# akloetgen/PARA-suite

Measured on AMD Instinct MI355X. Metric: aligned reads/sec (10Mx50bp PAR-CLIP vs hg19-size genome) on MI355X; SAM bit-exact vs own CPU restatement (parity unpinned), higher is better.
Workload: dtype u64

## Files before the change

para-suite_amd/csrc/ps_core.h:

```cpp
#pragma once
#include "ps_types.h"

namespace ps {

PS_HD uint32_t ps_popc(uint32_t x)
{
#ifdef __HIP_DEVICE_COMPILE__
    return (uint32_t)__popc(x);
#else
    return (uint32_t)__builtin_popcount(x);
#endif
}
PS_HD uint32_t pfx_mask32(int ns)
{
    return ns >= 32 ? 0xFFFFFFFFu : (ns <= 0 ? 0u : ((1u << ns) - 1u));
}

struct Blk { uint32_t x[16]; };

#ifdef __HIP_DEVICE_COMPILE__
#define PS_AS_GLOBAL(T, p) ((const __attribute__((address_space(1))) T *)(p))
#define PS_AS_GLOBAL_W(T, p) ((__attribute__((address_space(1))) T *)(p))
typedef uint32_t ps_u32x4 __attribute__((ext_vector_type(4)));
typedef uint32_t ps_u32x2 __attribute__((ext_vector_type(2)));
// ... 147 lines not shown
{
    if (base < 4) {
        uint32_t ok, ol;
        occ_pair1(ix, c.k, c.l, base, ok, ol, st);
        const bwtint l2 = L2_of(ix, base);
        c.k = l2 + ok + 1;
        c.l = l2 + ol;
    }
    if (c.k > c.l || base > 3) { c.k = 0; c.l = ix.seq_len; ++c.bid; }
    uint32_t w = width32(c.k, c.l);
    w_out = w;
    cw_out = cw_pack(c.bid, !first && w == c.prev_w);
    c.prev_w = w;
}

static const int PS_POP_TRIES = 1;
enum { M_FETCH = 0, M_POP = 1, M_EXACT = 2, M_EXPAND = 3, M_EXIT = 4, M_HIT = 5,
       M_GROW = 6 };

struct BtLane {
    int r, mode;
    bwtint k, l;
    int i, score, units, n_mm, n_gapo, n_gape, n_ins, n_del, state, ldp;
    bool have_cur;
    int best_score, max_units, n_aln, n_stack, status;
    unsigned long long best_cnt;
    unsigned long long bm0, bm1;
    uint32_t bump, free_head, iters0;
    uint32_t rn0, rn1;
    int len;
    uint32_t n_phantom;
    uint32_t cap;
    LaneStats st;
};

PS_HD int lm_ncw(int len) { return (len + 1 + 3) >> 2; }
PS_HD int lm_ncsw(int seed_len) { return seed_len > 0 ? (seed_len + 1 + 3) >> 2 : 0; }
PS_HD bool lm_nmask_in_regs(int len) { return len <= 64; }
PS_HD int lm_heads_off(int len, int seed_len) { return 4 * (lm_ncw(len) + lm_ncsw(seed_len) + ((len + 15) >> 4) + (lm_nmask_in_regs(len) ? 0 : ((len + 31) >> 5))); }
PS_HD int lm_bytes(int len, int seed_len, int n_buckets, bool wide)
{
    int n = lm_heads_off(len, seed_len) + (wide ? 0 : 2 * n_buckets);
    n = (n + 3) & ~3;
    if (((n >> 2) & 1) == 0) n += 4;
    return n;
}

static const int PS_JUMP_SLOT_WORDS = 8, PS_JUMP_MAX_LEVELS = 14;
PS_HD uint32_t jump_level_off(int d) { return 0x55555555u & ((1u << (2 * d)) - 1u); }
PS_HD size_t jump_words(int levels) { return (size_t)jump_level_off(levels) * PS_JUMP_SLOT_WORDS; }
PS_HD int jump_levels_for(bwtint seq_len) { int k = 0; while (k < PS_JUMP_MAX_LEVELS && (seq_len >> (2 * k)) >= 48) ++k; return k; }

static const int PS_CHASE_MIN2 = 16;
struct BtHot {
    const OccBlock *blocks; bwtint primary;
    const uint32_t *jump; uint32_t jump_levels;
    uint32_t skip_levels;
    uint32_t L2lo[4], L2hi;
    uint32_t s_pk[5], u_pk[5];
    uint32_t p0, p1, p2, p3;
    uint32_t inv_c_min, max_entries, pool_cap, n_reads, big_cap;
    uint32_t c_min;
    uint32_t chase;
    PS_HD int len() const { return (int)(p0 & 0xffu); }
    PS_HD int seed_len() const { return (int)((p0 >> 8) & 0xffu); }
    PS_HD int indel_end_skip() const { return (int)((p0 >> 16) & 0xffu); }
    PS_HD int max_del_occ() const { return (int)(p0 >> 24); }
    PS_HD int max_gapo() const { return (int)(p1 & 0xfu); }
    PS_HD int max_gape() const { return (int)((p1 >> 4) & 0xfu); }
    PS_HD bool mode_gape() const { return ((p1 >> 8) & 1u) != 0; }
    PS_HD bool use_seed() const { return ((p1 >> 9) & 1u) != 0; }
    PS_HD bool profile() const { return ((p1 >> 10) & 1u) != 0; }
    PS_HD bool has_big() const { return ((p1 >> 11) & 1u) != 0; }
    PS_HD int seed_units() const { return (int)((p1 >> 12) & 0xfffu); }
    PS_HD int u_tight() const { return (int)(p1 >> 24); }
    PS_HD int s_gapo_ins() const { return (int)(p2 & 0xffu); }
    PS_HD int s_gape() const { return (int)((p2 >> 8) & 0xffu); }
    PS_HD int s_gapo_del() const { return (int)((p2 >> 16) & 0xffu); }
    PS_HD int s_stop() const { return (int)(p2 >> 24); }
    PS_HD int u_gapo_ins() const { return (int)(p3 & 0xffu); }
    PS_HD int u_gape() const { return (int)((p3 >> 8) & 0xffu); }
    PS_HD int u_gapo_del() const { return (int)((p3 >> 16) & 0xffu); }
    PS_HD int n_buckets() const { return (int)(p3 >> 24); }
    PS_HD bwtint L2(int c) const
    { return (bwtint)L2lo[c] | ((bwtint)((L2hi >> c) & 1u) << 32); }
    PS_HD bwtint L2_dyn(int c) const
    { return (bwtint)sel4s(L2lo[0], L2lo[1], L2lo[2], L2lo[3], c) | ((bwtint)((L2hi >> c) & 1u) << 32); }
};
inline bool bt_hot_make(const BtArgs &a, BtHot &h)
{
    const Model &md = a.md;
    h.blocks = a.ix.blocks; h.primary = a.ix.primary; h.L2hi = 0;
    h.jump = a.ix.jump; h.jump_levels = a.ix.jump ? (uint32_t)a.ix.jump_levels : 0u;
    h.skip_levels = (a.no_skip || (((uint32_t)md.max_units * (uint32_t)md.inv_c_min) >> 16) > 127u) ? 0u : h.jump_levels;
    for (int c = 0; c < 4; ++c) { h.L2lo[c] = (uint32_t)a.ix.L2[c]; h.L2hi |= (uint32_t)((a.ix.L2[c] >> 32) & 1ull) << c; }
    h.L2hi |= (uint32_t)((a.ix.seq_len >> 32) & 1ull) << 4;
    for (int c = 0; c < 5; ++c) { h.s_pk[c] = md.s_mm_pk[c]; h.u_pk[c] = md.u_mm_pk[c]; }
    const int seed_units = md.max_seed_diff * md.u_tight;
    const bool ok = a.len >= 0 && a.len <= 255 && md.seed_len >= 0 && md.seed_len <= 255 && md.indel_end_skip >= 0 && md.indel_end_skip <= 255 &&
                    md.max_del_occ >= 0 && md.max_del_occ <= 255 && md.max_gapo >= 0 && md.max_gapo <= 15 && md.max_gape >= 0 && md.max_gape <= 15 &&
                    seed_units >= 0 && seed_units <= 4095 && md.u_tight >= 0 && md.u_tight <= 255 && md.s_stop >= 0 && md.s_stop <= 255 &&
                    md.s_gapo_ins >= 0 && md.s_gapo_ins <= 255 && md.s_gape >= 0 && md.s_gape <= 255 && md.s_gapo_del >= 0 && md.s_gapo_del <= 255 &&
                    md.u_gapo_ins >= 0 && md.u_gapo_ins <= 255 && md.u_gape >= 0 && md.u_gape <= 255 && md.u_gapo_del >= 0 && md.u_gapo_del <= 255 &&
                    md.n_buckets >= 0 && md.n_buckets <= 255 && md.max_entries >= 0 && md.inv_c_min >= 0 && md.max_units <= 255 && a.ix.L2[0] == 0;
    h.p0 = (uint32_t)a.len | ((uint32_t)md.seed_len << 8) | ((uint32_t)md.indel_end_skip << 16) | ((uint32_t)md.max_del_occ << 24);
    h.p1 = (uint32_t)md.max_gapo | ((uint32_t)md.max_gape << 4) | ((md.mode_gape ? 1u : 0u) << 8) | ((md.use_seed ? 1u : 0u) << 9) |
           ((md.profile ? 1u : 0u) << 10) | ((a.n_big ? 1u : 0u) << 11) | ((uint32_t)seed_units << 12) | ((uint32_t)md.u_tight << 24);
    h.p2 = (uint32_t)md.s_gapo_ins | ((uint32_t)md.s_gape << 8) | ((uint32_t)md.s_gapo_del << 16) | ((uint32_t)md.s_stop << 24);
    h.p3 = (uint32_t)md.u_gapo_ins | ((uint32_t)md.u_gape << 8) | ((uint32_t)md.u_gapo_del << 16) | ((uint32_t)md.n_buckets << 24);
    h.c_min = (uint32_t)md.c_min;
    h.chase = a.no_chase ? 0u : (uint32_t)(a.chase_min2 > 0 ? a.chase_min2 : PS_CHASE_MIN2);
    h.inv_c_min = (uint32_t)md.inv_c_min; h.max_entries = (uint32_t)md.max_entries; h.pool_cap = a.pool_cap; h.n_reads = (uint32_t)a.n_reads; h.big_cap = a.big_cap;
    return ok;
}

struct BtMem {
    uint8_t *cw, *csw;
    uint32_t *rb, *rn;
    uint16_t *heads16;
    void *pool;
    uint32_t *heads;
};

PS_HD void bt_mem_bind(BtMem &m, uint8_t *mine, int len, int seed_len)
{
    m.cw = mine; m.csw = mine + 4 * lm_ncw(len);
    m.rb = reinterpret_cast<uint32_t *>(m.csw + 4 * lm_ncsw(seed_len));
    m.rn = m.rb + ((len + 15) >> 4);
    m.heads16 = reinterpret_cast<uint16_t *>(mine + lm_heads_off(len, seed_len));
}
PS_HD int seq_at(const BtMem &m, const BtLane &L, int j, int len, int max_len)
{
    const int p = len - 1 - j;
    const uint32_t b = (m.rb[p >> 4] >> (2 * (p & 15))) & 3u;
    const uint32_t nw = lm_nmask_in_regs(max_len) ? (p < 32 ? L.rn0 : L.rn1) : m.rn[p >> 5];
    return ((nw >> (p & 31)) & 1u) ? 4 : 3 - (int)b;
}

struct Entry16 { uint32_t k, l, a, b; };
static const uint32_t PS_NIL16 = 0xFFFFu;

PS_HD bool bm_test(const BtLane &L, int b) { return (((b & 64) ? L.bm1 : L.bm0) >> (b & 63)) & 1ull; }
PS_HD void bm_set(BtLane &L, int b) { const unsigned long long v = 1ull << (b & 63); if (b & 64) L.bm1 |= v; else L.bm0 |= v; }
PS_HD void bm_clr(BtLane &L, int b) { const unsigned long long v = ~(1ull << (b & 63)); if (b & 64) L.bm1 &= v; else L.bm0 &= v; }
PS_HD int bm_first(const BtLane &L)
{
#ifdef __HIP_DEVICE_COMPILE__
    return L.bm0 ? (__ffsll((unsigned long long)L.bm0) - 1) : (64 + __ffsll((unsigned long long)L.bm1) - 1);
#else
    return L.bm0 ? __builtin_ctzll(L.bm0) : 64 + __builtin_ctzll(L.bm1);
#endif
}
PS_HD void store16(Entry16 *dst, const Entry16 &e)
{
#ifdef __HIP_DEVICE_COMPILE__
    ps_u32x4 v; v.x = e.k; v.y = e.l; v.z = e.a; v.w = e.b;
    *PS_AS_GLOBAL_W(ps_u32x4, dst) = v;
#else
    *dst = e;
#endif
}
PS_HD void load16(const Entry16 *src, Entry16 &e)
{
#ifdef __HIP_DEVICE_COMPILE__
// ... 346 lines not shown
```

para-suite_amd/csrc/ps_kernels.hip:

```cpp
#include <hip/hip_runtime.h>
#include <algorithm>
#include <cstdlib>
#include <stdexcept>
#include <string>
#include "ps_core.h"
#include "ps_narrow.h"
#include "ps_kernels.h"

namespace ps {

static const int PS_Q_CHUNK = 64;
#ifndef PS_BT_WAVES
#define PS_BT_WAVES 4
#endif

__device__ __forceinline__ unsigned long long wave_sum(unsigned long long v)
{
    for (int o = 32; o > 0; o >>= 1) v += __shfl_xor(v, o, 64);
    return v;
}
__device__ __forceinline__ void flush_stats(KStats *ks, const LaneStats &st)
{
    if (!ks) return;
    unsigned long long v[8] = {st.pairs, st.same, st.nodes, st.pushes, st.pops, st.lf, st.iters, st.exact};
// ... 21 lines not shown
        if (!seed_role) {
#pragma unroll 1
            for (int i = 0; i < len; ++i) {
                int j = len - 1 - i;
                if (i == 0 || (j & 15) == 15) bw = a.bases[(size_t)(j >> 4) * a.n_reads + opaque_lane(r)];
                if (i == 0 || (j & 31) == 31) mw = a.nmask[(size_t)(j >> 5) * a.n_reads + opaque_lane(r)];
                int base = ((mw >> (j & 31)) & 1u) ? 4 : (int)((bw >> (2 * (j & 15))) & 3u);
                uint32_t wv; uint8_t cb;
                wchain_step(a.ix, C, base, wv, cb, i == 0, st);
                a.w[(size_t)i * a.n_reads + opaque_lane(r)] = wv;
                cww |= (uint32_t)cb << (8 * (i & 3));
                if ((i & 3) == 3) { a.cwb[(size_t)(i >> 2) * a.n_reads + opaque_lane(r)] = cww; cww = 0; }
            }
            a.w[(size_t)len * a.n_reads + opaque_lane(r)] = 0;
            cww |= (uint32_t)cw_pack(C.bid + 1, false) << (8 * (len & 3));
            a.cwb[(size_t)(len >> 2) * a.n_reads + opaque_lane(r)] = cww;
        } else if (seeded) {
#pragma unroll 1
            for (int i = 0; i < seed_len; ++i) {
                int js = seed_len - 1 - i;
                if (i == 0 || (js & 15) == 15) bw = a.bases[(size_t)(js >> 4) * a.n_reads + opaque_lane(r)];
                if (i == 0 || (js & 31) == 31) mw = a.nmask[(size_t)(js >> 5) * a.n_reads + opaque_lane(r)];
                int sbase = ((mw >> (js & 31)) & 1u) ? 4 : (int)((bw >> (2 * (js & 15))) & 3u);
                uint32_t swv; uint8_t scb;
                wchain_step(a.ix, C, sbase, swv, scb, i == 0, st);
                cww |= (uint32_t)scb << (8 * (i & 3));
                if ((i & 3) == 3) { a.cswb[(size_t)(i >> 2) * a.n_reads + opaque_lane(r)] = cww; cww = 0; }
            }
            cww |= (uint32_t)cw_pack(C.bid + 1, false) << (8 * (seed_len & 3));
            a.cswb[(size_t)(seed_len >> 2) * a.n_reads + opaque_lane(r)] = cww;
        } else if (a.use_seed) {
            for (int p = 0; p <= (seed_len >> 2); ++p) a.cswb[(size_t)p * a.n_reads + opaque_lane(r)] = 0u;
        }
    }
    flush_stats(a.stats, st);
}

__device__ __forceinline__ uint32_t pin32(uint32_t v) { return (uint32_t)__builtin_amdgcn_readfirstlane((int)v); }
__device__ __forceinline__ unsigned long long pin64(unsigned long long v)
{
    return (unsigned long long)pin32((uint32_t)v) | ((unsigned long long)pin32((uint32_t)(v >> 32)) << 32);
}
__device__ __forceinline__ void pin_hot(BtHot &h, const BtHot &k)
{
    h.blocks = reinterpret_cast<const OccBlock *>(pin64(reinterpret_cast<unsigned long long>(k.blocks)));
    h.primary = pin64(k.primary);
    h.jump = reinterpret_cast<const uint32_t *>(pin64(reinterpret_cast<unsigned long long>(k.jump))); h.jump_levels = pin32(k.jump_levels); h.skip_levels = pin32(k.skip_levels);
#pragma unroll
    for (int c = 0; c < 4; ++c) h.L2lo[c] = pin32(k.L2lo[c]);
    h.L2hi = pin32(k.L2hi);
#pragma unroll
    for (int c = 0; c < 5; ++c) { h.s_pk[c] = pin32(k.s_pk[c]); h.u_pk[c] = pin32(k.u_pk[c]); }
    h.p0 = pin32(k.p0); h.p1 = pin32(k.p1); h.p2 = pin32(k.p2); h.p3 = pin32(k.p3);
    h.c_min = pin32(k.c_min); h.chase = pin32(k.chase);
    h.inv_c_min = pin32(k.inv_c_min); h.max_entries = pin32(k.max_entries); h.pool_cap = pin32(k.pool_cap); h.n_reads = pin32(k.n_reads); h.big_cap = pin32(k.big_cap);
}

__global__ void __launch_bounds__(256) k_backtrack_wide(const BtArgs *__restrict__ ap, BtHot hk, int lm_stride)
{
    const BtArgs &a = *ap;
    BtHot h; pin_hot(h, hk);
    uint32_t *const queue = reinterpret_cast<uint32_t *>(pin64(reinterpret_cast<unsigned long long>(a.queue)));
    const uint32_t n_reads = h.n_reads, fetch_min = pin32((uint32_t)a.fetch_min), hit_min = pin32((uint32_t)a.hit_min);
    extern __shared__ __attribute__((aligned(16))) uint8_t smem[];
    const int lane_g = blockIdx.x * blockDim.x + threadIdx.x;
    BtMem m;
    bt_mem_bind(m, smem + (size_t)threadIdx.x * lm_stride, h.len(), h.seed_len());
    m.pool = reinterpret_cast<uint8_t *>(a.pool) + (size_t)lane_g * h.pool_cap * sizeof(Entry);
    m.heads = a.heads + (size_t)lane_g * PS_MAX_BUCKETS;
    BtLane L;
    L.mode = M_FETCH; L.r = 0; L.have_cur = false; L.n_stack = 0; L.status = RS_OK; L.n_aln = 0;
    L.st = {0, 0, 0, 0, 0, 0, 0, 0};
    const int lane = threadIdx.x & 63;
    const unsigned long long lane_lt = (1ull << lane) - 1ull;
    const unsigned long long t_start = wall_clock64();
    int q_next = 0, q_end = 0;
    bool exhausted = false;
    for (;;) {
        const bool want = L.mode == M_FETCH;
        const unsigned long long wmask = __ballot(want), lmask = __ballot(L.mode != M_EXIT), hmask = __ballot(L.mode == M_HIT);
        if (lmask == 0) break;
        const bool stalled = (wmask | hmask) == lmask;
        const bool serve_hit = hmask != 0 && (__popcll(hmask) >= (int)hit_min || stalled);
        int fetch_r = -1;
        if (wmask) {
            const int cnt = __popcll(wmask);
            if (cnt >= (int)fetch_min || stalled) {
                const int rank = __popcll(wmask & lane_lt);
                int served = 0;
                while (served < cnt) {
                    if (q_next == q_end) {
                        if (exhausted) break;
                        unsigned int base = 0;
                        if (lane == 0) base = atomicAdd(queue, (unsigned int)PS_Q_CHUNK);
                        base = (unsigned int)__shfl((int)base, 0, 64);
                        if (base >= n_reads) { exhausted = true; break; }
                        q_next = (int)base;
                        q_end = (int)base + PS_Q_CHUNK < (int)n_reads ? (int)base + PS_Q_CHUNK : (int)n_reads;
                    }
                    const int take = q_end - q_next < cnt - served ? q_end - q_next : cnt - served;
                    if (want && rank >= served && rank < served + take) fetch_r = q_next + (rank - served);
                    q_next += take; served += take;
                }
                if (want && fetch_r < 0 && exhausted) fetch_r = (int)n_reads;
            }
        }
        bt_iter(a, h, L, m, fetch_r, serve_hit);
// ... 279 lines not shown
```

para-suite_amd/csrc/ps_narrow.h:

```cpp
#pragma once
#include "ps_core.h"

namespace ps {

PS_HD int nw_i(uint32_t wa) { return (int)(wa & 0xffu); }
PS_HD int nw_ldp(uint32_t wa) { return (int)((wa >> 8) & 0xffu); }
PS_HD int nw_mm(uint32_t wa) { return (int)((wa >> 16) & 0xffu); }
PS_HD int nw_state(uint32_t wa) { return (int)((wa >> 24) & 3u); }
PS_HD int nw_gapo(uint32_t wa) { return (int)((wa >> 26) & 7u); }
PS_HD int nw_gape(uint32_t wa) { return (int)(wa >> 29); }
PS_HD int nw_ins(uint32_t wb) { return (int)(wb & 7u); }
PS_HD int nw_del(uint32_t wb) { return (int)((wb >> 3) & 7u); }
PS_HD uint32_t nw_c(uint32_t wb) { return (wb >> 6) & 7u; }
PS_HD int nw_score(uint32_t wb) { return (int)((wb >> 9) & 0x7fu); }
static const uint32_t NW_KEEP = 0xFCFF0000u;
static const uint32_t NW_C_MASK = 7u << 6;
static const uint32_t NW_ROOT_C = 4u;

PS_HD int nl_mode(uint32_t ctl) { return (int)(ctl & 7u); }
PS_HD uint32_t nl_set_mode(uint32_t ctl, int mode) { return (ctl & ~7u) | (uint32_t)mode; }
static const uint32_t NL_HAVE_CUR = 8u, NL_STATUS = 7u << 4, NL_BIG = 1u << 7;
PS_HD int nl_status(uint32_t ctl) { return (int)((ctl >> 4) & 7u); }
PS_HD uint32_t nl_set_status(uint32_t ctl, int s) { return (ctl & ~NL_STATUS) | ((uint32_t)s << 4); }
PS_HD int nl_n_aln(uint32_t ctl) { return (int)(ctl >> 16); }
// ... 526 lines not shown

#ifndef PS_TABLE_SKIP
#define PS_TABLE_SKIP 1
#endif
static const int NT_SKIP_MAX = 4;
struct NtSkip { uint32_t ck, cl; };
static const uint32_t NT_NO_SKIP = 0xFFFFFFFFu;

PS_HD uint32_t nt_bytes_below(uint32_t hi, uint32_t lo, uint32_t e)
{
#ifdef __HIP_DEVICE_COMPILE__
    return __builtin_amdgcn_alignbyte(hi, lo, e & 3u);
#else
    const uint32_t sh = 8u * (e & 3u);
    return sh ? (hi << (32u - sh)) | (lo >> sh) : lo;
#endif
}
PS_HD uint32_t nt_bits_from(uint32_t hi, uint32_t lo, uint32_t sh)
{
#ifdef __HIP_DEVICE_COMPILE__
    return __builtin_amdgcn_alignbit(hi, lo, sh);
#else
    return sh ? (hi << (32u - sh)) | (lo >> sh) : lo;
#endif
}
PS_HD uint32_t nt_clz(uint32_t x)
{
#ifdef __HIP_DEVICE_COMPILE__
    return (uint32_t)__clz((int)x);
#else
    return x ? (uint32_t)__builtin_clz(x) : 32u;
#endif
}
PS_HD uint32_t nt_brev(uint32_t x)
{
#ifdef __HIP_DEVICE_COMPILE__
    return __brev(x);
#else
    x = ((x & 0x55555555u) << 1) | ((x >> 1) & 0x55555555u); x = ((x & 0x33333333u) << 2) | ((x >> 2) & 0x33333333u);
    x = ((x & 0x0f0f0f0fu) << 4) | ((x >> 4) & 0x0f0f0f0fu); x = ((x & 0x00ff00ffu) << 8) | ((x >> 8) & 0x00ff00ffu);
    return (x << 16) | (x >> 16);
#endif
}
PS_HD uint32_t nt_ge_key(int v)
{
    const uint32_t u = (uint32_t)(v > 128 ? 128 : v);
#ifdef __HIP_DEVICE_COMPILE__
    return 0x80808080u - __builtin_amdgcn_perm(u, u, 0u);
#else
    return 0x80808080u - u * 0x01010101u;
#endif
}

PS_HD int nt_skip(const BtHot &h, NLane &L, const BtMem &m, int mode, int rem, NtSkip &sk)
{
    sk.ck = NT_NO_SKIP; sk.cl = 0;
    const int len = nl_len(L), i1 = nw_i(L.wa);
    const int d = nt_depth(len, L.wa, L.wb);
    int t = (int)h.skip_levels - 1 - d;
    t = t > NT_SKIP_MAX ? NT_SKIP_MAX : t;
    t = t > i1 - 1 ? i1 - 1 : t;
    const int mleft = (int)(ps_mul24((uint32_t)rem, h.inv_c_min) >> 16);
    const uint32_t cap = (L.ctl & NL_BIG) ? h.big_cap : h.pool_cap;
    if (mode != M_EXPAND || t <= 0 || mleft == 0 || nl_bump(L) + 9u > cap) return mode;
    const uint32_t e = (uint32_t)(i1 - 1);
    const uint32_t *cw32 = reinterpret_cast<const uint32_t *>(m.cw);
    const int w0 = (int)(e >> 2);
    const uint32_t x0 = cw32[w0], x1 = cw32[w0 > 0 ? w0 - 1 : 0];
    const int r0 = len - i1;
    const int qb = r0 >> 4, qb_last = ((len + 15) >> 4) - 1;
    const uint32_t rb_lo = m.rb[qb], rb_hi = m.rb[qb < qb_last ? qb + 1 : qb_last];
    uint32_t nlo, nhi;
    if (lm_nmask_in_regs(h.len())) { const bool up = r0 >= 32; nlo = up ? L.rn1 : L.rn0; nhi = up ? 0u : L.rn1; }
    else { const int qn = r0 >> 5, qn_last = ((len + 31) >> 5) - 1; nlo = m.rn[qn]; nhi = m.rn[qn < qn_last ? qn + 1 : qn_last]; }
    const uint32_t sum = (nt_bytes_below(x0, x1, e) & 0x7f7f7f7fu) + nt_ge_key(mleft);
    uint32_t barren = sum & 0x80808080u;
    const uint32_t kills = (sum - 0x01010101u) & 0x80808080u;
    if (h.use_seed()) {
        const int off = len - h.seed_len(), ii = (int)e - off;
        const uint32_t vs = (uint32_t)((off > 0 && ii > 0) ? ii : 0);
        const int e_un = nl_max_units(L) - rem, srem = h.seed_units() - e_un;
        const int m_seed = srem <= 0 ? 0 : (int)(ps_mul24((uint32_t)srem, h.inv_c_min) >> 16);
        const uint32_t *cs32 = reinterpret_cast<const uint32_t *>(m.csw);
        const int s0 = (int)(vs >> 2);
        const uint32_t y0 = cs32[s0], y1 = cs32[s0 > 0 ? s0 - 1 : 0];
        const uint32_t valid = vs >= 4u ? 0xFFFFFFFFu : ~(0xFFFFFFFFu >> (8u * vs));
        barren |= ((nt_bytes_below(y0, y1, vs) & 0x7f7f7f7fu) + nt_ge_key(m_seed)) & valid & 0x80808080u;
    }
    const int run = (int)(nt_clz(barren ^ 0x80808080u) >> 3);
    t = t > run ? run : t;
    if (t == 0) return mode;
    const bool dead = (int)(nt_clz(kills) >> 3) < t || (nt_bits_from(nhi, nlo, (uint32_t)(r0 & 31)) & ((1u << t) - 1u)) != 0u;
    uint32_t y = nt_brev(nt_bits_from(rb_hi, rb_lo, (uint32_t)(2 * (r0 & 15))));
    y = ((y & 0x55555555u) << 1) | ((y >> 1) & 0x55555555u);
    const uint32_t sidx = (L.kr << (2 * t)) | (~y >> (32 - 2 * t));
    const uint32_t c = sidx & 3u;
    const uint32_t *ps = h.jump + (size_t)((jump_level_off(d + t - 1) + (sidx >> 2)) * (uint32_t)PS_JUMP_SLOT_WORDS + 2u * c);
#ifdef __HIP_DEVICE_COMPILE__
    const ps_u32x2 v = *PS_AS_GLOBAL(ps_u32x2, ps);
    sk.ck = v.x; sk.cl = v.y;
#else
    sk.ck = ps[0]; sk.cl = ps[1];
#endif
    L.kr = sidx;
    L.wa = (L.wa & NW_KEEP) + (uint32_t)(i1 - t);
    L.wb = (L.wb & ~NW_C_MASK) | (c << 6);
    if (dead) L.ctl = nl_set_mode(L.ctl, M_POP);
    return dead ? 0 : mode;
}
PS_HD int nt_skip_land(NLane &L, const NtSkip &sk, int mode)
{
    if (sk.ck == NT_NO_SKIP) return mode;
    if (sk.ck >= sk.cl) { L.ctl = nl_set_mode(L.ctl, M_POP); return 0; }
    L.lr = sk.cl - sk.ck;
    return mode;
}

template <bool STATS>
PS_HD bool nt_chase(const BtHot &h, NLane &L, LaneStats &st, const BtMem &m, const NtStep &q)
{
    const int i1 = nw_i(L.wa);
    if (!(L.ctl & NL_HAVE_CUR) || q.ctm || i1 < 2) return false;
    const int len = nl_len(L), i = i1 - 1;
    const int e_un = nt_units(h, L.wa, L.wb);
    const int mleft = (int)(ps_mul24((uint32_t)(nl_max_units(L) - e_un), h.inv_c_min) >> 16);
    const int ii = i - (len - h.seed_len());
    const bool in_seed = h.use_seed() && len > h.seed_len() && ii > 0;
    const int bnd = (int)(m.cw[i - 1] & 0x7f), s1 = in_seed ? (int)(m.csw[ii - 1] & 0x7f) : 0;
    const int s = nt_seq_at(m, L, i, len, h.len());
    if (mleft == 0 || s > 3 || !nt_barren(i, bnd, mleft, in_seed, s1, nt_m_seed(h, e_un))) return false;
    const bwtint base = nt_base(h, nw_c(L.wb));
    int ol_ = 0, ok_ = 0;
    const uint32_t bl = blk_of(row_to_stored(h.primary, base + L.lr), ol_), bk = blk_of(row_to_stored(h.primary, base + (bwtint)(L.kr - 1u)), ok_);
    if (bk != bl) return false;
    ++st.pairs; ++st.same;
    if (STATS) ++st.nodes;
    if (bnd > mleft) { L.ctl &= ~NL_HAVE_CUR; return false; }
    Blk x;
    load_blk(h.blocks, bl, x);
    const uint32_t ck = blk_count1b(x, ok_ + 1, s), cl = blk_count1b(x, ol_ + 1, s);
    if (ck >= cl) { L.ctl &= ~NL_HAVE_CUR; return false; }
    L.kr = ck + 1u; L.lr = cl; L.wa -= 1u; L.wb = (L.wb & ~NW_C_MASK) | ((uint32_t)s << 6);
    return true;
}

template <bool STATS, bool NB32>
PS_HD void nt_iter(const BtArgs &a, const BtHot &h, NLane &L, LaneStats &st, BtMem &m, int fetch_r, bool serve_hit, NtClock *clk = nullptr)
{
    PS_USTAMP(clk, 0);
    int rem = 0;
    int mode = nt_head<STATS, NB32>(a, h, L, st, m, fetch_r, serve_hit, rem);
    PS_USTAMP(clk, 1);
    NtSkip sk;
    sk.ck = NT_NO_SKIP;
    if (PS_TABLE_SKIP && mode) mode = nt_skip(h, L, m, mode, rem, sk);
    NtStep q;
    if (mode) nt_step_occ<STATS>(h, L, st, m, q);
    if (PS_TABLE_SKIP) mode = nt_skip_land(L, sk, mode);
#if PS_TABLE_SKIP && defined(__HIP_DEVICE_COMPILE__)
    asm volatile("" : "+v"(L.kr), "+v"(L.lr), "+v"(L.wa), "+v"(L.wb), "+v"(L.ctl), "+v"(mode));
#endif
#if defined(PS_STAMPS) && defined(__HIP_DEVICE_COMPILE__)
    if (STATS && clk && mode) asm volatile("" :: "v"(q.ck[0]), "v"(q.cl[0]), "v"(q.ck[3]), "v"(q.cl[3]));
#endif
    PS_USTAMP(clk, 2);
    bool barren = false;
    if (mode) barren = nt_tail<STATS, NB32>(h, L, st, m, q, mode);
    bool chased = false;
    if (PS_CHASE && h.chase != 0u && barren) chased = nt_chase<STATS>(h, L, st, m, q);
#if PS_CHASE
    {
#ifdef __HIP_DEVICE_COMPILE__
        const bool enough = __popcll(__ballot(chased)) >= (int)h.chase;
#else
        const bool enough = h.chase <= 64u;
#endif
        if (enough && chased) nt_chase<STATS>(h, L, st, m, q);
    }
#endif
    (void)chased;
    PS_USTAMP(clk, 3);
}

}
```

para-suite_amd/csrc/ps_search.hip:

```cpp
#include <hip/hip_runtime.h>
#include <hipcub/hipcub.hpp>
#include <algorithm>
#include <cstring>
#include <optional>
#include "ps_pipeline.h"
#include "ps_search_plan.h"
#include "ps_dev.h"
#include "ps_par.h"

namespace ps {

__global__ void k_gather_alns(const AlnRec *alns, int aln_cap, const int32_t *n_aln, const uint32_t *off, int n, AlnRec *out)
{
    for (int r = blockIdx.x * blockDim.x + threadIdx.x; r < n; r += gridDim.x * blockDim.x) {
        int m = n_aln[r]; if (m > aln_cap) m = aln_cap;
        for (int j = 0; j < m; ++j) out[off[r] + j] = alns[(size_t)r * aln_cap + j];
    }
}
__global__ void k_clip_counts(const int32_t *n_aln, int aln_cap, int n, uint32_t *out)
{
    for (int r = blockIdx.x * blockDim.x + threadIdx.x; r < n; r += gridDim.x * blockDim.x) { int m = n_aln[r]; out[r] = (uint32_t)(m > aln_cap ? aln_cap : (m < 0 ? 0 : m)); }
}

__global__ void k_order_keys(const uint8_t *est, int n, int cap, uint8_t *key)
// ... 39 lines not shown
        em.n_reads = n; em.len = a.len; em.lens = a.lens; em.units_by_len = a.units_by_len; em.bases = a.bases; em.nmask = a.nmask; em.cwb = a.cwb; em.est = est;
        for (int c = 0; c < 5; ++c) em.s_pk[c] = md.u_mm_pk[c];
        em.inv_c_min = (uint32_t)md.inv_c_min; em.max_units = md.max_units; em.u_tight = md.u_tight;
        em.seed_units = md.max_seed_diff * md.u_tight; em.use_seed = md.use_seed; em.seed_len = md.seed_len;
        em.max_gapo = md.max_gapo; em.indel_end_skip = md.indel_end_skip; em.u_gapo_ins = md.u_gapo_ins; em.u_gapo_del = md.u_gapo_del;
        em.depth = lv + 3; em.rows = (float)a.ix.seq_len; em.log_scale = kn.order_scale;
        em.key = key; em.pred = nullptr;
        launch_effort_model(em, s);
    }
    launch_order_sort(key, n, wk->ws_get<uint32_t>("order_tmp", order_sort_tmp_words(n)), order, s);
    PS_HIP(hipGetLastError());
    t->stop(s);
    a.order = order; a.est = est; a.est_ab = ea.est_ab;
}

static const uint8_t *upload_units_by_len(Batch &b)
{
    uint8_t *tab = b.wk->pin_get<uint8_t>("units_by_len_h", 256), *d_tab = b.wk->ws_get<uint8_t>("units_by_len", 256);
    budget_units_by_len(b.ctx->opt, tab);
    PS_HIP(hipMemcpyAsync(d_tab, tab, 256, hipMemcpyHostToDevice, b.wk->stream));
    return d_tab;
}

static SearchPlan search_stacks(Batch &b, BtArgs &a, const SearchKnobs &kn, int lm)
{
    Ctx *ctx = b.ctx; Work *wk = b.wk; hipStream_t s = wk->stream;
    const SearchPlan p = plan_search(a.n_reads, lm, a.pool_cap, a.wide != 0, ctx->cus, ctx->bt_blocks, kn.max_per_cu, ctx->n_big);
    a.n_lanes = p.lanes;
    a.pool = wk->ws_get<uint8_t>("pool", p.pool_bytes);
    a.heads = a.wide ? wk->ws_get<uint32_t>("heads", p.head_words) : nullptr;
    a.queue = wk->ws_get<uint32_t>("queue", 16);
    PS_HIP(hipMemsetAsync(a.queue, 0, 64, s));
    if (p.n_big) {
        a.big_cap = PS_BIG_CAP; a.n_big = p.n_big;
        a.big_pool = wk->ws_get<uint8_t>("big_pool", p.big_bytes);
        a.big_next = a.queue + 4;
        a.big_busy = wk->ws_get<uint32_t>("big_busy", a.n_big);
        PS_HIP(hipMemsetAsync(a.big_busy, 0, (size_t)a.n_big * 4, s));
    }
    return p;
}

static void run_search(Batch &b, const SearchKnobs &kn, const Model &md, int n, const uint32_t *d_bases, const uint32_t *d_nmask, const int32_t *d_lens,
                       uint32_t pool_cap, int aln_cap, AlnRec *alns, int32_t *n_aln, uint8_t *status, bool first_tier = false)
{
    Ctx *ctx = b.ctx; Work *wk = b.wk; hipStream_t s = wk->stream;
    const int len = md.len;
    const bool wide = launch_is_wide(md, pool_cap);
    BtArgs a; std::memset(&a, 0, sizeof a);
    a.ix = ctx->ix.view; a.md = md; a.n_reads = n; a.len = len; a.lens = d_lens;
    a.bases = d_bases; a.nmask = d_nmask; a.n_bw = (len + 15) / 16; a.n_mw = (len + 31) / 32;
    a.alns = alns; a.aln_cap = aln_cap; a.n_aln = n_aln; a.status = status;
    a.pool_cap = pool_cap; a.wide = wide ? 1 : 0; a.stats = b.d_stats.p + 1; a.fetch_min = kn.fetch_min; a.hit_min = kn.hit_min;
    a.no_skip = kn.skip ? 0 : 1; a.no_chase = kn.chase ? 0 : 1; a.chase_min2 = kn.chase_min2;
    EventPair t_width; std::optional<EventPair> t_order;
    search_width(b, a, t_width);
    if (d_lens) a.units_by_len = upload_units_by_len(b);
    search_order(b, a, kn, t_order);
    a.cap_est = (first_tier && !wide && a.est && md.profile && kn.cap) ? 1 + kn.cap_bias : 0;
    const int lm = lm_bytes(len, md.seed_len, md.n_buckets, wide);
    const SearchPlan p = search_stacks(b, a, kn, lm);
    if (ctx->want_read_iters) { a.read_iters = wk->ws_get<uint32_t>("riters", (size_t)n * PS_RI_WORDS); PS_HIP(hipMemsetAsync(a.read_iters, 0, (size_t)n * PS_RI_WORDS * 4, s)); }
    EventPair t(s);
    if (!launch_backtrack(a, wk->ws_get<BtArgs>("btargs", 1), wk->pin_get<BtArgs>("btargs_h", 1), p.blocks, lm, s, ctx->want_kstats || ctx->want_read_iters)) throw Error("cost model outside the ranges the search kernel packs (gap/score fields must fit a byte)");
    PS_HIP(hipGetLastError());
    t.stop(s);
    const double ms = t.ms(); b.tm.ms_backtrack += ms; ++b.tm.n_backtrack_launches;
    b.tm.ms_width += t_width.ms();
    if (t_order) b.tm.ms_width += t_order->ms();
    { double t0_ = 0, t1_ = 0; t.span(ctx->ref_event, t0_, t1_); if (b.tm.n_backtrack_launches == 1) b.tm.bt_begin_ms = t0_; b.tm.bt_end_ms = t1_; }
    if (std::getenv("PS_VERBOSE")) std::fprintf(stderr, "[parasuite-hip]   backtrack launch: %d reads x %d bp, stack %u%s, %d lanes, %.1f ms\n", n, len, pool_cap, wide ? " (wide)" : "", p.lanes, ms);
    if (ctx->want_read_iters) { ctx->read_iters.resize((size_t)n * PS_RI_WORDS); PS_HIP(hipMemcpyAsync(ctx->read_iters.data(), a.read_iters, (size_t)n * PS_RI_WORDS * 4, hipMemcpyDeviceToHost, s)); PS_HIP(hipStreamSynchronize(s)); }
}

static void download_alns(Work *wk, int n, int aln_cap, const AlnRec *d_alns, const int32_t *d_n_aln,
                          std::vector<int32_t> &n_aln, std::vector<uint32_t> &off, std::vector<AlnRec> &alns)
{
    hipStream_t s = wk->stream;
    uint32_t *cnt = wk->ws_get<uint32_t>("cnt", n), *d_off = wk->ws_get<uint32_t>("off", (size_t)n + 1);
    hipLaunchKernelGGL(k_clip_counts, dim3((n + 255) / 256), dim3(256), 0, s, d_n_aln, aln_cap, n, cnt);
    size_t tb = 0;
    PS_HIP(hipcub::DeviceScan::ExclusiveSum(nullptr, tb, cnt, d_off, n, s));
    uint8_t *tmp = wk->ws_get<uint8_t>("scan_tmp", tb ? tb : 1);
    PS_HIP(hipcub::DeviceScan::ExclusiveSum(tmp, tb, cnt, d_off, n, s));
    int32_t *p_na = wk->pin_get<int32_t>("dl_n_aln", n); uint32_t *p_off = wk->pin_get<uint32_t>("dl_off", (size_t)n + 1);
    PS_HIP(hipMemcpyAsync(p_na, d_n_aln, (size_t)n * 4, hipMemcpyDeviceToHost, s));
    PS_HIP(hipMemcpyAsync(p_off, d_off, (size_t)n * 4, hipMemcpyDeviceToHost, s));
    PS_HIP(hipStreamSynchronize(s));
    uint32_t last = 0;
    if (n) { int m = p_na[n - 1]; last = p_off[n - 1] + (uint32_t)(m > aln_cap ? aln_cap : (m < 0 ? 0 : m)); }
    p_off[n] = last;
    n_aln.assign(p_na, p_na + n); off.assign(p_off, p_off + n + 1); alns.resize(last);
    if (last) {
        AlnRec *comp = wk->ws_get<AlnRec>("comp", last);
        hipLaunchKernelGGL(k_gather_alns, dim3((n + 255) / 256), dim3(256), 0, s, d_alns, aln_cap, d_n_aln, d_off, n, comp);
        AlnRec *p_al = wk->pin_get<AlnRec>("dl_alns", last);
        PS_HIP(hipMemcpyAsync(p_al, comp, (size_t)last * sizeof(AlnRec), hipMemcpyDeviceToHost, s));
        PS_HIP(hipStreamSynchronize(s));
        std::memcpy(alns.data(), p_al, (size_t)last * sizeof(AlnRec));
    }
}

__global__ void k_classify(const AlnRec *alns, int aln_cap, const int32_t *n_aln, const uint8_t *status, const int32_t *ids,
                           int n, int n_occ, uint8_t *cls_out)
{
    for (int r = blockIdx.x * blockDim.x + threadIdx.x; r < n; r += gridDim.x * blockDim.x) {
        uint8_t c = 0;
// ... 212 lines not shown
```

para-suite_amd/csrc/ps_search_plan.h:

```cpp
#pragma once
#include <algorithm>
#include <cstdint>
#include <cstdlib>
#include "ps_budget.h"
#include "ps_core.h"
#include "ps_error.h"
#include "ps_model.h"

namespace ps {

struct SearchKnobs {
    int order = 1, order_min = 4096, order_restart = 0 , order_wpin = 16, order_cap = 255, order_scale = 8;
    int max_per_cu = PS_SEARCH_WAVES;
    bool cap = true; int cap_bias = 0;
    bool skip = true;
    int chase_min2 = PS_CHASE_MIN2;
    bool chase = true;
    int fetch_min = 8, hit_min = 1;
};
inline SearchKnobs search_knobs_from_env(int ctx_fetch_min, int ctx_hit_min)
{
    SearchKnobs k; int v = 0;
    k.fetch_min = ctx_fetch_min; k.hit_min = ctx_hit_min;
    if (env_int("PS_ORDER", v)) k.order = v;
    if (env_int("PS_ORDER_MIN", v)) k.order_min = std::max(1, v);
    if (env_int("PS_ORDER_RESTART", v)) k.order_restart = std::max(1, v);
    if (env_int("PS_ORDER_WPIN", v)) k.order_wpin = std::max(1, v);
    if (env_int("PS_ORDER_CAP", v)) k.order_cap = std::max(1, std::min(255, v));
    if (env_int("PS_ORDER_SCALE", v)) k.order_scale = std::max(1, std::min(12, v));
    if (env_int("PS_MAX_PER_CU", v)) k.max_per_cu = v;
    if (env_int("PS_CAP", v)) k.cap = v != 0;
    if (env_int("PS_CAP_BIAS", v)) k.cap_bias = std::max(0, std::min(200, v));
    if (env_int("PS_SKIP", v)) k.skip = v != 0;
    if (env_int("PS_CHASE", v)) k.chase = v != 0;
    if (env_int("PS_CHASE_MIN2", v)) k.chase_min2 = std::max(1, std::min(65, v));
    if (env_int("PS_FETCH_MIN", v)) k.fetch_min = std::max(1, v);
    if (env_int("PS_HIT_MIN", v)) k.hit_min = std::max(1, v);
    return k;
}

struct SearchPlan { int blocks = 0, lanes = 0; size_t pool_bytes = 0, head_words = 0; uint32_t n_big = 0; size_t big_bytes = 0; };
static const uint32_t PS_BIG_CAP = 65535;
inline SearchPlan plan_search(int64_t n_reads, int lm_bytes_per_lane, uint32_t pool_cap, bool wide, int cus, int bt_blocks, int max_per_cu, int n_big)
{
    int per_cu = (int)(PS_CU_LDS / ((size_t)256 * lm_bytes_per_lane));
    if (per_cu < 1) throw Error("read length / score range too large for the per-lane LDS state");
    if (bt_blocks <= 0 && max_per_cu < 1) throw Error("PS_MAX_PER_CU must be at least 1");
    int64_t blocks = std::min<int64_t>(bt_blocks > 0 ? bt_blocks : (int64_t)cus * std::min(per_cu, max_per_cu), (n_reads + 255) / 256);
    const size_t entry = wide ? sizeof(Entry) : sizeof(Entry16), per_lane = (size_t)pool_cap * entry + (wide ? PS_MAX_BUCKETS * 4 : 0);
    const size_t max_lanes = ((size_t)(wide ? 32 : 64) << 30) / per_lane;
    if ((size_t)blocks * 256 > max_lanes) blocks = (int64_t)std::max<size_t>(1, max_lanes / 256);
    SearchPlan p;
    p.blocks = (int)blocks; p.lanes = p.blocks * 256;
    p.pool_bytes = (size_t)p.lanes * pool_cap * entry;
    p.head_words = wide ? (size_t)p.lanes * PS_MAX_BUCKETS : 0;
    if (!wide && pool_cap < PS_BIG_CAP && n_big > 0) {
        p.n_big = (uint32_t)std::min<int64_t>(n_big, std::max<int64_t>(64, n_reads));
        p.big_bytes = (size_t)p.n_big * PS_BIG_CAP * sizeof(Entry16);
    }
    return p;
}
inline SearchPlan plan_search_reserve(uint32_t pool_cap, int cus, int bt_blocks, int n_big)
{
    if (pool_cap > PS_BIG_CAP) return SearchPlan();
    return plan_search(INT32_MAX, (int)PS_SEARCH_LDS_PER_LANE, pool_cap, false, cus, bt_blocks, PS_SEARCH_WAVES, n_big);
}

inline void budget_units_by_len(const Options &o, uint8_t tab[256])
{
    for (int l = 0; l < 256; ++l) { const int u = budget_diffs(o, l) * (o.profile ? o.unit : 1); tab[l] = (uint8_t)(u > 255 ? 255 : u); }
}

}
```

para-suite_amd/csrc/ps_types.h:

```cpp
#pragma once
#include <stdint.h>
#include <stddef.h>

#ifdef __HIPCC__
#define PS_HD __host__ __device__ __forceinline__
#define PS_COLD __host__ __device__ inline __attribute__((noinline))
#else
#define PS_HD inline
#define PS_COLD inline
#endif

namespace ps {

typedef uint64_t bwtint;
static const bwtint PS_MAX_ROWS = (1ull << 33) - 64;

static const int PS_BLK_SYMS = 192;
struct OccBlock { uint32_t cnt[4]; uint32_t sym[12]; };

struct IndexView {
    const OccBlock *blocks;
    const uint32_t *sa;
    const uint32_t *sa_hi;
    const uint8_t  *pac;
// ... 11 lines not shown
    uint8_t u_mm[5][4], s_mm[5][4];
    uint32_t u_mm_pk[5], s_mm_pk[5];
    int32_t u_gapo_ins, s_gapo_ins, u_gapo_del, s_gapo_del, u_gape, s_gape;
    int32_t s_stop, u_tight, c_min, inv_c_min , max_units, n_buckets;
    int32_t max_gapo, max_gape, mode_gape, indel_end_skip, max_del_occ, max_entries;
    int32_t seed_len, max_seed_diff, max_top2, use_seed, len, profile;
};
static const int PS_MAX_BUCKETS = 128;
static const int PS_MAX_LEN = 250;

struct Entry {
    bwtint k, l;
    uint16_t score, units;
    uint8_t i, last_diff_pos, n_mm, n_gapo, n_gape, n_ins, n_del, state;
    uint32_t next;
};
static const uint32_t PS_NIL = 0xFFFFFFFFu;
enum { ST_M = 0, ST_I = 1, ST_D = 2 };

struct AlnRec {
    bwtint k, l;
    uint16_t score, units;
    uint8_t n_mm, n_gapo, n_gape, n_ins, n_del, pad[7];
};

enum { RS_OK = 0, RS_OVERFLOW_POOL = 1, RS_OVERFLOW_ALN = 2, RS_BAD_SCORE = 3,
       RS_OVERFLOW_DEEP = 4 };

struct KStats {
    unsigned long long occ_pairs, occ_same_blk, nodes, pushes, pops, lf_steps, iters, exact_steps;
};

static const int PS_RI_WORDS = 20;
struct BtArgs {
    IndexView ix;
    Model md;
    int n_reads, len, n_lanes;
    const int32_t *lens;
    const uint8_t *units_by_len;
    const uint32_t *bases; const uint32_t *nmask; int n_bw, n_mw;
    uint32_t *w; const uint32_t *cwb; const uint32_t *cswb;
    AlnRec *alns; int aln_cap; int32_t *n_aln; uint8_t *status;
    void *pool; uint32_t pool_cap;
    uint32_t *heads;
    int wide;
    uint8_t *big_pool; uint32_t big_cap, n_big; uint32_t *big_busy; uint32_t *big_next;
    uint32_t *queue;
    const int32_t *order;
    const uint8_t *est; const uint16_t *est_ab;
    int cap_est;
    int no_skip;
    int no_chase;
    int chase_min2;
    uint32_t *read_iters;
    int hit_min;
    int fetch_min;
    KStats *stats;
};

}
```

Measured before the change: 9.847 million.

## Extend jump-table skip and same-block chase to exact-match search mode

Lets the lane in exact-match mode advance several symbols at once, either through the precomputed jump table (skip) or through single-block occurrence chasing. Previously these shortcuts only applied in expand mode. The goal is to cut per-symbol LF-mapping steps and occ-block fetches during exact extension. Both paths are on by default and gated by an env knob and a compile-time macro. This adds branching and register pressure in the hot step loop, and the empty-interval and termination handling in exact mode must stay bit-exact.

```diff
diff --git a/para-suite_amd/csrc/ps_core.h b/para-suite_amd/csrc/ps_core.h
--- a/para-suite_amd/csrc/ps_core.h
+++ b/para-suite_amd/csrc/ps_core.h
@@ -223,6 +223,9 @@
 PS_HD int jump_levels_for(bwtint seq_len) { int k = 0; while (k < PS_JUMP_MAX_LEVELS && (seq_len >> (2 * k)) >= 48) ++k; return k; }
 
 static const int PS_CHASE_MIN2 = 16;
+#ifndef PS_EXACT_RUN
+#define PS_EXACT_RUN 2
+#endif
 struct BtHot {
     const OccBlock *blocks; bwtint primary;
     const uint32_t *jump; uint32_t jump_levels;
@@ -233,6 +236,7 @@
     uint32_t inv_c_min, max_entries, pool_cap, n_reads, big_cap;
     uint32_t c_min;
     uint32_t chase;
+    uint32_t exact_run;
     PS_HD int len() const { return (int)(p0 & 0xffu); }
     PS_HD int seed_len() const { return (int)((p0 >> 8) & 0xffu); }
     PS_HD int indel_end_skip() const { return (int)((p0 >> 16) & 0xffu); }
@@ -281,6 +285,7 @@
     h.p3 = (uint32_t)md.u_gapo_ins | ((uint32_t)md.u_gape << 8) | ((uint32_t)md.u_gapo_del << 16) | ((uint32_t)md.n_buckets << 24);
     h.c_min = (uint32_t)md.c_min;
     h.chase = a.no_chase ? 0u : (uint32_t)(a.chase_min2 > 0 ? a.chase_min2 : PS_CHASE_MIN2);
+    h.exact_run = ((PS_EXACT_RUN > 0 && a.exact_off < 2 && h.skip_levels) ? 1u : 0u) | ((PS_EXACT_RUN > 1 && a.exact_off < 1 && h.chase) ? 2u : 0u);
     h.inv_c_min = (uint32_t)md.inv_c_min; h.max_entries = (uint32_t)md.max_entries; h.pool_cap = a.pool_cap; h.n_reads = (uint32_t)a.n_reads; h.big_cap = a.big_cap;
     return ok;
 }
diff --git a/para-suite_amd/csrc/ps_kernels.hip b/para-suite_amd/csrc/ps_kernels.hip
--- a/para-suite_amd/csrc/ps_kernels.hip
+++ b/para-suite_amd/csrc/ps_kernels.hip
@@ -97,7 +97,7 @@
 #pragma unroll
     for (int c = 0; c < 5; ++c) { h.s_pk[c] = pin32(k.s_pk[c]); h.u_pk[c] = pin32(k.u_pk[c]); }
     h.p0 = pin32(k.p0); h.p1 = pin32(k.p1); h.p2 = pin32(k.p2); h.p3 = pin32(k.p3);
-    h.c_min = pin32(k.c_min); h.chase = pin32(k.chase);
+    h.c_min = pin32(k.c_min); h.chase = pin32(k.chase); h.exact_run = pin32(k.exact_run);
     h.inv_c_min = pin32(k.inv_c_min); h.max_entries = pin32(k.max_entries); h.pool_cap = pin32(k.pool_cap); h.n_reads = pin32(k.n_reads); h.big_cap = pin32(k.big_cap);
 }
 
diff --git a/para-suite_amd/csrc/ps_narrow.h b/para-suite_amd/csrc/ps_narrow.h
--- a/para-suite_amd/csrc/ps_narrow.h
+++ b/para-suite_amd/csrc/ps_narrow.h
@@ -602,7 +602,8 @@
 #endif
 }
 
-PS_HD int nt_skip(const BtHot &h, NLane &L, const BtMem &m, int mode, int rem, NtSkip &sk)
+template <bool STATS>
+PS_HD int nt_skip(const BtHot &h, NLane &L, LaneStats &st, const BtMem &m, int mode, int rem, NtSkip &sk)
 {
     sk.ck = NT_NO_SKIP; sk.cl = 0;
     const int len = nl_len(L), i1 = nw_i(L.wa);
@@ -612,7 +613,13 @@
     t = t > i1 - 1 ? i1 - 1 : t;
     const int mleft = (int)(ps_mul24((uint32_t)rem, h.inv_c_min) >> 16);
     const uint32_t cap = (L.ctl & NL_BIG) ? h.big_cap : h.pool_cap;
+#if PS_EXACT_RUN
+    const bool ex = mode == M_EXACT && (h.exact_run & 1u) != 0u;
+    if (t <= 0 || !(ex || (mode == M_EXPAND && mleft != 0 && nl_bump(L) + 9u <= cap))) return mode;
+#else
+    const bool ex = false;
     if (mode != M_EXPAND || t <= 0 || mleft == 0 || nl_bump(L) + 9u > cap) return mode;
+#endif
     const uint32_t e = (uint32_t)(i1 - 1);
     const uint32_t *cw32 = reinterpret_cast<const uint32_t *>(m.cw);
     const int w0 = (int)(e >> 2);
@@ -625,7 +632,8 @@
     else { const int qn = r0 >> 5, qn_last = ((len + 31) >> 5) - 1; nlo = m.rn[qn]; nhi = m.rn[qn < qn_last ? qn + 1 : qn_last]; }
     const uint32_t sum = (nt_bytes_below(x0, x1, e) & 0x7f7f7f7fu) + nt_ge_key(mleft);
     uint32_t barren = sum & 0x80808080u;
-    const uint32_t kills = (sum - 0x01010101u) & 0x80808080u;
+    uint32_t kills = (sum - 0x01010101u) & 0x80808080u;
+    if (ex) kills = 0u;
     if (h.use_seed()) {
         const int off = len - h.seed_len(), ii = (int)e - off;
         const uint32_t vs = (uint32_t)((off > 0 && ii > 0) ? ii : 0);
@@ -637,6 +645,7 @@
         const uint32_t valid = vs >= 4u ? 0xFFFFFFFFu : ~(0xFFFFFFFFu >> (8u * vs));
         barren |= ((nt_bytes_below(y0, y1, vs) & 0x7f7f7f7fu) + nt_ge_key(m_seed)) & valid & 0x80808080u;
     }
+    if (ex) barren = 0x80808080u;
     const int run = (int)(nt_clz(barren ^ 0x80808080u) >> 3);
     t = t > run ? run : t;
     if (t == 0) return mode;
@@ -652,8 +661,17 @@
 #else
     sk.ck = ps[0]; sk.cl = ps[1];
 #endif
+    if (STATS && ex) {
+        const uint32_t nbits = nt_bits_from(nhi, nlo, (uint32_t)(r0 & 31));
+        for (int j = 1; j <= t; ++j) {
+            ++st.exact;
+            const uint32_t sj = sidx >> (2 * (t - j));
+            const uint32_t *pj = h.jump + (size_t)((jump_level_off(d + j - 1) + (sj >> 2)) * (uint32_t)PS_JUMP_SLOT_WORDS + 2u * (sj & 3u));
+            if (((nbits >> (j - 1)) & 1u) || pj[0] >= pj[1]) break;
+        }
+    }
     L.kr = sidx;
-    L.wa = (L.wa & NW_KEEP) + (uint32_t)(i1 - t);
+    L.wa = ex ? L.wa - (uint32_t)t : (L.wa & NW_KEEP) + (uint32_t)(i1 - t);
     L.wb = (L.wb & ~NW_C_MASK) | (c << 6);
     if (dead) L.ctl = nl_set_mode(L.ctl, M_POP);
     return dead ? 0 : mode;
@@ -670,27 +688,29 @@
 PS_HD bool nt_chase(const BtHot &h, NLane &L, LaneStats &st, const BtMem &m, const NtStep &q)
 {
     const int i1 = nw_i(L.wa);
-    if (!(L.ctl & NL_HAVE_CUR) || q.ctm || i1 < 2) return false;
+    const bool ex = PS_EXACT_RUN && (h.exact_run & 2u) != 0u && nl_mode(L.ctl) == M_EXACT;
+    if (!(ex || (L.ctl & NL_HAVE_CUR)) || q.ctm || i1 < (ex ? 1 : 2)) return false;
     const int len = nl_len(L), i = i1 - 1;
     const int e_un = nt_units(h, L.wa, L.wb);
     const int mleft = (int)(ps_mul24((uint32_t)(nl_max_units(L) - e_un), h.inv_c_min) >> 16);
     const int ii = i - (len - h.seed_len());
     const bool in_seed = h.use_seed() && len > h.seed_len() && ii > 0;
-    const int bnd = (int)(m.cw[i - 1] & 0x7f), s1 = in_seed ? (int)(m.csw[ii - 1] & 0x7f) : 0;
+    const int bnd = (int)(m.cw[(PS_EXACT_RUN && i < 1) ? 0 : i - 1] & 0x7f), s1 = in_seed ? (int)(m.csw[ii - 1] & 0x7f) : 0;
     const int s = nt_seq_at(m, L, i, len, h.len());
-    if (mleft == 0 || s > 3 || !nt_barren(i, bnd, mleft, in_seed, s1, nt_m_seed(h, e_un))) return false;
+    if ((!ex && mleft == 0) || s > 3 || (!ex && !nt_barren(i, bnd, mleft, in_seed, s1, nt_m_seed(h, e_un)))) return false;
     const bwtint base = nt_base(h, nw_c(L.wb));
     int ol_ = 0, ok_ = 0;
     const uint32_t bl = blk_of(row_to_stored(h.primary, base + L.lr), ol_), bk = blk_of(row_to_stored(h.primary, base + (bwtint)(L.kr - 1u)), ok_);
     if (bk != bl) return false;
     ++st.pairs; ++st.same;
-    if (STATS) ++st.nodes;
-    if (bnd > mleft) { L.ctl &= ~NL_HAVE_CUR; return false; }
+    if (STATS) { if (ex) ++st.exact; else ++st.nodes; }
+    if (!ex && bnd > mleft) { L.ctl &= ~NL_HAVE_CUR; return false; }
     Blk x;
     load_blk(h.blocks, bl, x);
     const uint32_t ck = blk_count1b(x, ok_ + 1, s), cl = blk_count1b(x, ol_ + 1, s);
-    if (ck >= cl) { L.ctl &= ~NL_HAVE_CUR; return false; }
+    if (ck >= cl) { L.ctl = ex ? nl_set_mode(L.ctl, M_POP) : L.ctl & ~NL_HAVE_CUR; return false; }
     L.kr = ck + 1u; L.lr = cl; L.wa -= 1u; L.wb = (L.wb & ~NW_C_MASK) | ((uint32_t)s << 6);
+    if (ex && i == 0) { L.ctl = nl_set_mode(L.ctl, M_HIT); return false; }
     return true;
 }
 
@@ -703,7 +723,7 @@
     PS_USTAMP(clk, 1);
     NtSkip sk;
     sk.ck = NT_NO_SKIP;
-    if (PS_TABLE_SKIP && mode) mode = nt_skip(h, L, m, mode, rem, sk);
+    if (PS_TABLE_SKIP && mode) mode = nt_skip<STATS>(h, L, st, m, mode, rem, sk);
     NtStep q;
     if (mode) nt_step_occ<STATS>(h, L, st, m, q);
     if (PS_TABLE_SKIP) mode = nt_skip_land(L, sk, mode);
@@ -717,6 +737,7 @@
     bool barren = false;
     if (mode) barren = nt_tail<STATS, NB32>(h, L, st, m, q, mode);
     bool chased = false;
+    if (PS_EXACT_RUN && (h.exact_run & 2u) != 0u && nl_mode(L.ctl) == M_EXACT) barren = true;
     if (PS_CHASE && h.chase != 0u && barren) chased = nt_chase<STATS>(h, L, st, m, q);
 #if PS_CHASE
     {
diff --git a/para-suite_amd/csrc/ps_search.hip b/para-suite_amd/csrc/ps_search.hip
--- a/para-suite_amd/csrc/ps_search.hip
+++ b/para-suite_amd/csrc/ps_search.hip
@@ -115,7 +115,7 @@
     a.bases = d_bases; a.nmask = d_nmask; a.n_bw = (len + 15) / 16; a.n_mw = (len + 31) / 32;
     a.alns = alns; a.aln_cap = aln_cap; a.n_aln = n_aln; a.status = status;
     a.pool_cap = pool_cap; a.wide = wide ? 1 : 0; a.stats = b.d_stats.p + 1; a.fetch_min = kn.fetch_min; a.hit_min = kn.hit_min;
-    a.no_skip = kn.skip ? 0 : 1; a.no_chase = kn.chase ? 0 : 1; a.chase_min2 = kn.chase_min2;
+    a.no_skip = kn.skip ? 0 : 1; a.no_chase = kn.chase ? 0 : 1; a.chase_min2 = kn.chase_min2; a.exact_off = 2 - kn.exact_run;
     EventPair t_width; std::optional<EventPair> t_order;
     search_width(b, a, t_width);
     if (d_lens) a.units_by_len = upload_units_by_len(b);
diff --git a/para-suite_amd/csrc/ps_search_plan.h b/para-suite_amd/csrc/ps_search_plan.h
--- a/para-suite_amd/csrc/ps_search_plan.h
+++ b/para-suite_amd/csrc/ps_search_plan.h
@@ -16,6 +16,7 @@
     bool skip = true;
     int chase_min2 = PS_CHASE_MIN2;
     bool chase = true;
+    int exact_run = 2;
     int fetch_min = 8, hit_min = 1;
 };
 inline SearchKnobs search_knobs_from_env(int ctx_fetch_min, int ctx_hit_min)
@@ -34,6 +35,7 @@
     if (env_int("PS_SKIP", v)) k.skip = v != 0;
     if (env_int("PS_CHASE", v)) k.chase = v != 0;
     if (env_int("PS_CHASE_MIN2", v)) k.chase_min2 = std::max(1, std::min(65, v));
+    if (env_int("PS_EXACT_RUN", v)) k.exact_run = std::max(0, std::min(2, v));
     if (env_int("PS_FETCH_MIN", v)) k.fetch_min = std::max(1, v);
     if (env_int("PS_HIT_MIN", v)) k.hit_min = std::max(1, v);
     return k;
diff --git a/para-suite_amd/csrc/ps_types.h b/para-suite_amd/csrc/ps_types.h
--- a/para-suite_amd/csrc/ps_types.h
+++ b/para-suite_amd/csrc/ps_types.h
@@ -87,6 +87,7 @@
     int no_skip;
     int no_chase;
     int chase_min2;
+    int exact_off;
     uint32_t *read_iters;
     int hit_min;
     int fetch_min;
```

Result: slower. 9.586 million (-2.7%).
